# gnosisguild/stylus-zkvm-verifiers

Measured on AMD Instinct MI355X. Metric: Groth16 proofs verified/sec (BN254), higher is better.
Workload: dtype u32

## Files before the change

### stylus_zkvm_verifiers_amd/csrc/zkv_field.h

```cpp
#pragma once
#include <stdint.h>
#include "bn254_constants.h"

#if defined(__HIPCC__)
#define ZKV_HD __host__ __device__ __forceinline__
#define ZKV_HD_NI __host__ __device__ __noinline__ inline
#else
#define ZKV_HD inline
#define ZKV_HD_NI inline
#endif

#if defined(ZKV_COUNT_FP_MUL)
static thread_local unsigned long long zkv_fp_mul_counter = 0;
static thread_local unsigned long long zkv_mad_counter = 0;
#define ZKV_COUNT_MADS(n) (zkv_mad_counter += (n))
#else
#define ZKV_COUNT_MADS(n) ((void)0)
#endif

#if defined(__HIP_DEVICE_COMPILE__)
#define ZKV_TABLE static __device__ const
#else
#define ZKV_TABLE static const
#endif

#if defined(ZKV_ASM_MARKS) && defined(__HIP_DEVICE_COMPILE__)
#define ZKV_MARK(name) asm volatile("; ZKVMARK " name)
#else
#define ZKV_MARK(name) ((void)0)
#endif

#ifndef ZKV_FAIR_SLICE_SHIFT
#define ZKV_FAIR_SLICE_SHIFT 17
#endif
ZKV_HD uint32_t zkv_wave_slot_parity() {
#if defined(__HIP_DEVICE_COMPILE__) && !defined(ZKV_NO_FAIR_SHARE)
    return __builtin_amdgcn_s_getreg((3 << 11) | 4) & 1u;
#else
    return 0;
#endif
}
ZKV_HD void zkv_fair_share(uint32_t slot_parity) {
#if defined(__HIP_DEVICE_COMPILE__) && !defined(ZKV_NO_FAIR_SHARE)
    const uint32_t t = (uint32_t)(__builtin_amdgcn_s_memrealtime() >> ZKV_FAIR_SLICE_SHIFT);
    if ((t ^ slot_parity) & 1u) __builtin_amdgcn_s_setprio(1);
    else __builtin_amdgcn_s_setprio(0);
#else
    (void)slot_parity;
#endif
}

#include "zkv_modinv.h"

namespace zkv {

struct Fp { uint32_t v[8]; };
struct Fp2C { Fp c0, c1; };
#if defined(ZKV_PAIRED)
struct Fp2 { Fp h; };
#else
struct Fp2 { Fp c0, c1; };
#endif
struct Fp6 { Fp2 c0, c1, c2; };

#if defined(__has_builtin)
#if __has_builtin(__builtin_addc) && __has_builtin(__builtin_subc)
#define ZKV_HAVE_CARRY_BUILTINS 1
#endif
#endif
ZKV_HD uint32_t addc(uint32_t a, uint32_t b, uint32_t& carry) {
#if defined(ZKV_HAVE_CARRY_BUILTINS)
    unsigned co; uint32_t r = __builtin_addc(a, b, carry, &co); carry = co; return r;
#else
    uint64_t t = (uint64_t)a + b + carry;
    carry = (uint32_t)(t >> 32);
    return (uint32_t)t;
#endif
}
ZKV_HD uint32_t subb(uint32_t a, uint32_t b, uint32_t& borrow) {
#if defined(ZKV_HAVE_CARRY_BUILTINS)
    unsigned bo; uint32_t r = __builtin_subc(a, b, borrow, &bo); borrow = bo; return r;
#else
    uint64_t t = (uint64_t)a - b - borrow;
    borrow = (uint32_t)(t >> 32) & 1u;
    return (uint32_t)t;
#endif
}

ZKV_HD Fp fp_zero() { Fp r; for (int i = 0; i < 8; i++) r.v[i] = 0; return r; }
ZKV_HD Fp fp_one() { Fp r = ZKV_FP_ONE; return r; }
ZKV_HD bool fp_is_zero(const Fp& a) {
    const uint32_t P[8] = ZKV_FP_P_LIMBS;
    uint32_t o = 0, q = 0;
    for (int i = 0; i < 8; i++) { o |= a.v[i]; q |= a.v[i] ^ P[i]; }
    return o == 0 || q == 0;
}
ZKV_HD bool u256_geq(const uint32_t* a, const uint32_t* m) {
    uint32_t br = 0;
    for (int i = 0; i < 8; i++) (void)subb(a[i], m[i], br);
    return br == 0;
}
ZKV_HD Fp fp_add(const Fp& a, const Fp& b) {
    const uint32_t P[8] = ZKV_FP_2P_LIMBS;
    Fp t, s; uint32_t c = 0, br = 0;
#pragma unroll
    for (int i = 0; i < 8; i++) t.v[i] = addc(a.v[i], b.v[i], c);
#pragma unroll
    for (int i = 0; i < 8; i++) s.v[i] = subb(t.v[i], P[i], br);
#pragma unroll
    for (int i = 0; i < 8; i++) t.v[i] = br ? t.v[i] : s.v[i];
    return t;
}
ZKV_HD Fp fp_sub(const Fp& a, const Fp& b) {
    const uint32_t P[8] = ZKV_FP_2P_LIMBS;
    Fp t; uint32_t br = 0, c = 0;
#pragma unroll
    for (int i = 0; i < 8; i++) t.v[i] = subb(a.v[i], b.v[i], br);
    uint32_t mask = 0u - br;
#pragma unroll
    for (int i = 0; i < 8; i++) t.v[i] = addc(t.v[i], P[i] & mask, c);
    return t;
}
ZKV_HD bool fp_eq(const Fp& a, const Fp& b) { return fp_is_zero(fp_sub(a, b)); }
ZKV_HD Fp fp_neg(const Fp& a) { return fp_sub(fp_zero(), a); }
ZKV_HD Fp fp_dbl(const Fp& a) { return fp_add(a, a); }
ZKV_HD Fp fp_half(const Fp& a) {
    const uint32_t P[8] = ZKV_FP_P_LIMBS;
    const uint32_t m = 0u - (a.v[0] & 1u);
    Fp t; uint32_t c = 0;
#pragma unroll
    for (int i = 0; i < 8; i++) t.v[i] = addc(a.v[i], P[i] & m, c);
    Fp r;
#pragma unroll
    for (int i = 0; i < 7; i++) r.v[i] = (t.v[i] >> 1) | (t.v[i + 1] << 31);
    r.v[7] = t.v[7] >> 1;
    return r;
}
ZKV_HD Fp fp_add_nr(const Fp& a, const Fp& b) {
    Fp t; uint32_t c = 0;
#pragma unroll
    for (int i = 0; i < 8; i++) t.v[i] = addc(a.v[i], b.v[i], c);
    return t;
}
ZKV_HD void fp_add_x2(const Fp& a0, const Fp& b0, const Fp& a1, const Fp& b1, Fp& r0, Fp& r1) {
    const uint32_t P[8] = ZKV_FP_2P_LIMBS;
    Fp t0, t1, s0, s1; uint32_t c0 = 0, c1 = 0, w0 = 0, w1 = 0;
#pragma unroll
    for (int i = 0; i < 8; i++) { t0.v[i] = addc(a0.v[i], b0.v[i], c0); t1.v[i] = addc(a1.v[i], b1.v[i], c1); }
#pragma unroll
    for (int i = 0; i < 8; i++) { s0.v[i] = subb(t0.v[i], P[i], w0); s1.v[i] = subb(t1.v[i], P[i], w1); }
#pragma unroll
    for (int i = 0; i < 8; i++) { r0.v[i] = w0 ? t0.v[i] : s0.v[i]; r1.v[i] = w1 ? t1.v[i] : s1.v[i]; }
}
ZKV_HD void fp_sub_x2(const Fp& a0, const Fp& b0, const Fp& a1, const Fp& b1, Fp& r0, Fp& r1) {
    const uint32_t P[8] = ZKV_FP_2P_LIMBS;
    Fp t0, t1; uint32_t w0 = 0, w1 = 0, c0 = 0, c1 = 0;
#pragma unroll
    for (int i = 0; i < 8; i++) { t0.v[i] = subb(a0.v[i], b0.v[i], w0); t1.v[i] = subb(a1.v[i], b1.v[i], w1); }
    uint32_t m0 = 0u - w0, m1 = 0u - w1;
#pragma unroll
    for (int i = 0; i < 8; i++) { r0.v[i] = addc(t0.v[i], P[i] & m0, c0); r1.v[i] = addc(t1.v[i], P[i] & m1, c1); }
}

ZKV_HD void fp_unpack29(const Fp& a, uint32_t x[9]) {
#pragma unroll
    for (int k = 0; k < 9; k++) {
        const int bit = 29 * k, w = bit >> 5, s = bit & 31;
        uint32_t v = a.v[w] >> s;
        if (s > 3 && w < 7) v |= a.v[w + 1] << (32 - s);
        x[k] = v & 0x1fffffffu;
    }
}
template <typename COL>
ZKV_HD void fp_mac81(COL col[18], const uint32_t x[9], const uint32_t y[9]) {
    ZKV_COUNT_MADS(81);
#pragma unroll
    for (int i = 0; i < 9; i++) {
#pragma unroll
        for (int j = 0; j < 9; j++) col[i + j] = (COL)((uint64_t)col[i + j] + (uint64_t)x[i] * y[j]);
    }
}
template <typename COL>
ZKV_HD void fp_reduce_cols_limbs(COL col[18], uint32_t (&r)[9]) {
    ZKV_COUNT_MADS(81);
    const uint32_t P29[9] = ZKV_FP_P29_LIMBS;
    const uint32_t M29 = 0x1fffffffu;
#pragma unroll
    for (int i = 0; i < 9; i++) {
        uint32_t m = ((uint32_t)col[i] * ZKV_FP_INV29) & M29;
#pragma unroll
        for (int j = 0; j < 9; j++) col[i + j] = (COL)((uint64_t)col[i + j] + (uint64_t)m * P29[j]);
        col[i + 1] += col[i] >> 29;
    }
#pragma unroll
    for (int k = 9; k < 17; k++) {
        r[k - 9] = (uint32_t)col[k] & M29;
        col[k + 1] += col[k] >> 29;
    }
    r[8] = (uint32_t)col[17];
}
ZKV_HD Fp fp_pack29(const uint32_t (&r)[9]) {
    Fp o;
#pragma unroll
    for (int w = 0; w < 8; w++) {
        const int bit = 32 * w, k = bit / 29, s = bit - 29 * k, got = 29 - s;
        uint32_t v = r[k] >> s;
        if (k + 1 < 9) v |= r[k + 1] << got;
        if (got + 29 < 32 && k + 2 < 9) v |= r[k + 2] << (got + 29);
        o.v[w] = v;
    }
    return o;
}
template <typename COL>
ZKV_HD Fp fp_reduce_cols(COL col[18]) {
    uint32_t r[9];
    fp_reduce_cols_limbs(col, r);
    return fp_pack29(r);
}
#if defined(ZKV_FP_MUL_NOINLINE)
ZKV_HD_NI
#else
ZKV_HD
#endif
Fp fp_mul(Fp a, Fp b) {
#if defined(ZKV_COUNT_FP_MUL)
    zkv_fp_mul_counter++;
#endif
    uint32_t x[9], y[9];
    fp_unpack29(a, x); fp_unpack29(b, y);
    int64_t col[18];
#pragma unroll
    for (int k = 0; k < 18; k++) col[k] = 0;
    fp_mac81(col, x, y);
    return fp_reduce_cols(col);
}
#if defined(ZKV_FP_MUL_NOINLINE)
ZKV_HD_NI
#else
ZKV_HD
#endif
Fp fp_sqr(Fp a) {
#if defined(ZKV_COUNT_FP_MUL)
    zkv_fp_mul_counter++;
#endif
    uint32_t x[9], d[9];
    fp_unpack29(a, x);
#pragma unroll
    for (int i = 0; i < 9; i++) d[i] = x[i] << 1;
    uint64_t col[18];
    ZKV_COUNT_MADS(45);
#pragma unroll
    for (int k = 0; k < 18; k++) col[k] = 0;
#pragma unroll
    for (int i = 0; i < 9; i++) {
        col[2 * i] += (uint64_t)x[i] * x[i];
#pragma unroll
        for (int j = i + 1; j < 9; j++) col[i + j] += (uint64_t)d[i] * x[j];
    }
    return fp_reduce_cols(col);
}

ZKV_HD Fp fp_from_raw(const uint32_t* limbs) {
    Fp t, r2 = ZKV_FP_R2;
    for (int i = 0; i < 8; i++) t.v[i] = limbs[i];
    return fp_mul(t, r2);
}
ZKV_HD void fp_to_raw(uint32_t* limbs, const Fp& a) {
    const uint32_t P[8] = ZKV_FP_P_LIMBS;
    Fp one = fp_zero(); one.v[0] = 1;
    Fp t = fp_mul(a, one), s; uint32_t br = 0;
    for (int i = 0; i < 8; i++) s.v[i] = subb(t.v[i], P[i], br);
    for (int i = 0; i < 8; i++) limbs[i] = br ? t.v[i] : s.v[i];
}
ZKV_HD Fp fp_inv_fermat(const Fp& a) {
    const uint8_t S[ZKV_FP_INV_SCHED_LEN] = ZKV_FP_INV_SCHED;
    const Fp a3 = fp_mul(fp_sqr(a), a);
    Fp acc = (S[0] & 7) == 3 ? a3 : a;
#pragma unroll 1
    for (int i = 1; i < ZKV_FP_INV_SCHED_LEN; i++) {
        const int nsq = S[i] >> 3, v = S[i] & 7;
#pragma unroll 1
        for (int k = 0; k < nsq; k++) acc = fp_sqr(acc);
        if (v) {
            Fp m;
#pragma unroll
            for (int k = 0; k < 8; k++) m.v[k] = v == 3 ? a3.v[k] : a.v[k];
            acc = fp_mul(acc, m);
        }
    }
    return acc;
}

ZKV_HD Fp fp_inv(const Fp& a) {
    const int32_t M[9] = ZKV_FP_M30_LIMBS;
    const Fp r3 = ZKV_FP_R3;
    Fp t = a;
    modinv30(t.v, M, ZKV_FP_MINV30);
    return fp_mul(t, r3);
}

template <int N>
ZKV_HD void fp_add_n(const Fp (&a)[N], const Fp (&b)[N], Fp (&r)[N]) {
    const uint32_t P[8] = ZKV_FP_2P_LIMBS;
    Fp t[N], s[N]; uint32_t c[N], w[N];
#pragma unroll
    for (int k = 0; k < N; k++) { c[k] = 0; w[k] = 0; }
#pragma unroll
    for (int i = 0; i < 8; i++) {
#pragma unroll
        for (int k = 0; k < N; k++) t[k].v[i] = addc(a[k].v[i], b[k].v[i], c[k]);
    }
#pragma unroll
    for (int i = 0; i < 8; i++) {
#pragma unroll
        for (int k = 0; k < N; k++) s[k].v[i] = subb(t[k].v[i], P[i], w[k]);
    }
#pragma unroll
    for (int i = 0; i < 8; i++) {
#pragma unroll
        for (int k = 0; k < N; k++) r[k].v[i] = w[k] ? t[k].v[i] : s[k].v[i];
    }
}
template <int N>
ZKV_HD void fp_sub_n(const Fp (&a)[N], const Fp (&b)[N], Fp (&r)[N]) {
    const uint32_t P[8] = ZKV_FP_2P_LIMBS;
    Fp t[N]; uint32_t w[N], c[N], m[N];
#pragma unroll
    for (int k = 0; k < N; k++) { c[k] = 0; w[k] = 0; }
#pragma unroll
    for (int i = 0; i < 8; i++) {
#pragma unroll
        for (int k = 0; k < N; k++) t[k].v[i] = subb(a[k].v[i], b[k].v[i], w[k]);
    }
#pragma unroll
    for (int k = 0; k < N; k++) m[k] = 0u - w[k];
#pragma unroll
    for (int i = 0; i < 8; i++) {
#pragma unroll
        for (int k = 0; k < N; k++) r[k].v[i] = addc(t[k].v[i], P[i] & m[k], c[k]);
    }
// ... 81 lines not shown
    Fp r;
#pragma unroll
    for (int i = 0; i < 8; i++) r.v[i] = zkv_partner_u32(a.v[i]);
    return r;
}
ZKV_HD Fp fp_sel(bool odd, const Fp& if_odd, const Fp& if_even) {
    Fp r;
#pragma unroll
    for (int i = 0; i < 8; i++) r.v[i] = odd ? if_odd.v[i] : if_even.v[i];
    return r;
}
ZKV_HD Fp2 f2_const(const Fp2C& c) { Fp2 r; r.h = fp_sel(zkv_parity() != 0, c.c1, c.c0); return r; }
ZKV_HD Fp2 f2_zero() { Fp2 r; r.h = fp_zero(); return r; }
ZKV_HD Fp2 f2_one() { Fp2 r; r.h = fp_sel(zkv_parity() != 0, fp_zero(), fp_one()); return r; }
ZKV_HD bool f2_is_zero(const Fp2& a) {
    uint32_t o = fp_is_zero(a.h) ? 0u : 1u;
    o |= zkv_partner_u32(o);
    return o == 0;
}
ZKV_HD bool f2_eq(const Fp2& a, const Fp2& b) {
    uint32_t o = fp_eq(a.h, b.h) ? 0u : 1u;
    o |= zkv_partner_u32(o);
    return o == 0;
}
ZKV_HD Fp2 f2_add(const Fp2& a, const Fp2& b) { Fp2 r; r.h = fp_add(a.h, b.h); return r; }
ZKV_HD Fp2 f2_sub(const Fp2& a, const Fp2& b) { Fp2 r; r.h = fp_sub(a.h, b.h); return r; }
ZKV_HD Fp2 f2_neg(const Fp2& a) { Fp2 r; r.h = fp_neg(a.h); return r; }
ZKV_HD Fp2 f2_add_nr(const Fp2& a, const Fp2& b) { Fp2 r; r.h = fp_add_nr(a.h, b.h); return r; }
ZKV_HD Fp2 f2_dbl(const Fp2& a) { return f2_add(a, a); }
ZKV_HD Fp2 f2_half(const Fp2& a) { Fp2 r; r.h = fp_half(a.h); return r; }
ZKV_HD Fp2 f2_conj(const Fp2& a) { Fp2 r; r.h = fp_sel(zkv_parity() != 0, fp_neg(a.h), a.h); return r; }
#if defined(ZKV_FP_MUL_NOINLINE)
ZKV_HD_NI
#else
ZKV_HD
#endif
Fp f2_mul_lane(Fp my_a, Fp my_b) {
#if defined(ZKV_COUNT_FP_MUL)
    zkv_fp_mul_counter += 2;
#endif
    const uint32_t FAT[9] = ZKV_FP_FAT8P_LIMBS;
    const bool odd = zkv_parity() != 0;
    uint32_t xa[9], xo[9], yb[9], U[9], V[9];
    fp_unpack29(my_a, xa); fp_unpack29(my_b, yb);
#pragma unroll
    for (int i = 0; i < 9; i++) { xo[i] = zkv_partner_u32(xa[i]); U[i] = zkv_pair_even_u32(yb[i]); V[i] = zkv_pair_odd_u32(yb[i]); }
    if (!odd) {
#pragma unroll
        for (int i = 0; i < 9; i++) V[i] = FAT[i] - V[i];
    }
    uint64_t col[18];
#pragma unroll
    for (int k = 0; k < 18; k++) col[k] = 0;
    fp_mac81(col, xa, U); fp_mac81(col, xo, V);
    return fp_reduce_cols(col);
}
ZKV_HD Fp2 f2_mul(const Fp2& a, const Fp2& b) { Fp2 r; r.h = f2_mul_lane(a.h, b.h); return r; }
ZKV_HD void f2_limbs_x(const Fp& v, uint32_t (&own)[9], uint32_t (&par)[9]) {
    fp_unpack29(v, own);
#pragma unroll
    for (int i = 0; i < 9; i++) par[i] = zkv_partner_u32(own[i]);
}
ZKV_HD void f2_limbs_y(const Fp& v, uint32_t (&U)[9], uint32_t (&V)[9]) {
    const uint32_t FAT[9] = ZKV_FP_FAT8P_LIMBS;
    uint32_t y[9];
    fp_unpack29(v, y);
#pragma unroll
    for (int i = 0; i < 9; i++) { U[i] = zkv_pair_even_u32(y[i]); V[i] = zkv_pair_odd_u32(y[i]); }
    if (zkv_parity() == 0) {
#pragma unroll
        for (int i = 0; i < 9; i++) V[i] = FAT[i] - V[i];
    }
}
ZKV_HD Fp f2_dot2_limbs(const uint32_t (&ao)[9], const uint32_t (&ap)[9], const uint32_t (&bU)[9], const uint32_t (&bV)[9],
                        const uint32_t (&co)[9], const uint32_t (&cp)[9], const uint32_t (&dU)[9], const uint32_t (&dV)[9]) {
#if defined(ZKV_COUNT_FP_MUL)
    zkv_fp_mul_counter += 4;
#endif
    uint64_t col[18];
#pragma unroll
    for (int k = 0; k < 18; k++) col[k] = 0;
    fp_mac81(col, ao, bU); fp_mac81(col, ap, bV); fp_mac81(col, co, dU); fp_mac81(col, cp, dV);
    return fp_reduce_cols(col);
}
ZKV_HD Fp f2_mul_limbs(const uint32_t (&ao)[9], const uint32_t (&ap)[9], const uint32_t (&bU)[9], const uint32_t (&bV)[9]) {
#if defined(ZKV_COUNT_FP_MUL)
    zkv_fp_mul_counter += 2;
#endif
    uint64_t col[18];
#pragma unroll
    for (int k = 0; k < 18; k++) col[k] = 0;
    fp_mac81(col, ao, bU); fp_mac81(col, ap, bV);
    return fp_reduce_cols(col);
}
struct L9 { uint32_t l[9]; };
ZKV_HD L9 l9_from_fp(const Fp& a) { L9 r; fp_unpack29(a, r.l); return r; }
ZKV_HD Fp l9_to_fp(const L9& a) { return fp_pack29(a.l); }
ZKV_HD L9 l9_partner(const L9& a) {
    L9 r;
#pragma unroll
    for (int i = 0; i < 9; i++) r.l[i] = zkv_partner_u32(a.l[i]);
    return r;
}
ZKV_HD L9 l9_mul_core(const L9& a, const L9& b) {
#if defined(ZKV_COUNT_FP_MUL)
    zkv_fp_mul_counter += 2;
#endif
    const uint32_t FAT[9] = ZKV_FP_FAT8P_LIMBS;
    uint32_t xo[9], U[9], V[9];
    uint64_t col[18];
#pragma unroll
    for (int k = 0; k < 18; k++) col[k] = 0;
#pragma unroll
    for (int i = 0; i < 9; i++) U[i] = zkv_pair_even_u32(b.l[i]);
    fp_mac81(col, a.l, U);
#pragma unroll
    for (int i = 0; i < 9; i++) { xo[i] = zkv_partner_u32(a.l[i]); V[i] = zkv_pair_odd_u32(b.l[i]); }
    if (zkv_parity() == 0) {
#pragma unroll
        for (int i = 0; i < 9; i++) V[i] = FAT[i] - V[i];
    }
    fp_mac81(col, xo, V);
    L9 r; fp_reduce_cols_limbs(col, r.l);
    return r;
}
#if defined(__HIP_DEVICE_COMPILE__) && defined(ZKV_FP_MUL_NOINLINE)
#define ZKV_L9P(p) uint32_t p##0, uint32_t p##1, uint32_t p##2, uint32_t p##3, uint32_t p##4, uint32_t p##5, uint32_t p##6, uint32_t p##7, uint32_t p##8
#define ZKV_L9A(f) f.l[0], f.l[1], f.l[2], f.l[3], f.l[4], f.l[5], f.l[6], f.l[7], f.l[8]
#define ZKV_L9MK(f, p) L9 f; f.l[0] = p##0; f.l[1] = p##1; f.l[2] = p##2; f.l[3] = p##3; f.l[4] = p##4; f.l[5] = p##5; f.l[6] = p##6; f.l[7] = p##7; f.l[8] = p##8
__device__ __noinline__ inline L9 l9_mul_ni(ZKV_L9P(pa), ZKV_L9P(pb)) {
    ZKV_L9MK(a, pa); ZKV_L9MK(b, pb);
    return l9_mul_core(a, b);
}
ZKV_HD L9 l9_mul(const L9& a, const L9& b) { return l9_mul_ni(ZKV_L9A(a), ZKV_L9A(b)); }
#else
ZKV_HD L9 l9_mul(const L9& a, const L9& b) { return l9_mul_core(a, b); }
#endif
struct LTerm { const uint32_t* x; int32_t k; };
#define ZKV_L9_G 256
template <int N> ZKV_HD L9 l9_lincomb(const LTerm (&t)[N], const int c) {
    const uint32_t P29[9] = ZKV_FP_P29_LIMBS;
    const int32_t D = (int32_t)P29[8] + 1;
    const uint32_t M = (uint32_t)(((1ull << 53) + (uint64_t)D - 1) / (uint64_t)D);
    int32_t top = 0;
#pragma unroll
    for (int j = 0; j < N; j++) top += t[j].k * (int32_t)t[j].x[8];
    const uint32_t tt = (uint32_t)(top + c * D - c - ZKV_L9_G);
    const int32_t nq = c - (int32_t)(uint32_t)(((uint64_t)tt * M) >> 53);
    L9 y; int64_t carry = 0;
#pragma unroll
    for (int i = 0; i < 9; i++) {
        int64_t s = carry;
#pragma unroll
        for (int j = 0; j < N; j++) s += (int64_t)t[j].k * (int64_t)(int32_t)t[j].x[i];
        s += (int64_t)nq * (int64_t)(int32_t)P29[i];
        if (i < 8) { y.l[i] = (uint32_t)s & 0x1fffffffu; carry = s >> 29; }
        else y.l[i] = (uint32_t)s;
    }
    return y;
}
ZKV_HD Fp2 f2_sqr(const Fp2& a) {
    const bool odd = zkv_parity() != 0;
    Fp o = zkv_partner(a.h);
    Fp x = fp_add_nr(a.h, fp_sel(odd, a.h, o));
    Fp y = fp_sel(odd, o, fp_sub(a.h, o));
    Fp2 r; r.h = fp_mul(x, y);
// ... 94 lines not shown
```

### stylus_zkvm_verifiers_amd/csrc/zkv_tower_mem.h

```cpp
#pragma once
#include "zkv_curve.h"

namespace zkv {

struct MRef {
    uint32_t* p; uint32_t stride; uint32_t f2w;
    ZKV_HD uint32_t ld(int k) const { return p[(size_t)k * stride]; }
    ZKV_HD void st(int k, uint32_t v) const { p[(size_t)k * stride] = v; }
    ZKV_HD int fw() const { return (int)f2w; }
};
ZKV_HD MRef m_ref(uint32_t* p, uint32_t stride, uint32_t f2w = 16) { MRef r; r.p = p; r.stride = stride; r.f2w = f2w; return r; }
ZKV_HD MRef m_off(MRef m, int words) { MRef r = m; r.p = m.p + (size_t)words * m.stride; return r; }

struct SoaRW {
    uint32_t* p; size_t stride; uint32_t off;
    ZKV_HD uint32_t ld(int k) const { return *(const uint32_t*)((const char*)(p + (size_t)k * stride) + off); }
    ZKV_HD void st(int k, uint32_t v) const { *(uint32_t*)((char*)(p + (size_t)k * stride) + off) = v; }
    ZKV_HD int fw() const { return 16; }
};
template <class R> ZKV_HD R m_fresh(R r) { return r; }
ZKV_HD SoaRW m_fresh(SoaRW r) {
#if defined(__HIP_DEVICE_COMPILE__)
    asm volatile("" : "+v"(r.off));
#endif
    return r;
}

#if defined(__HIP_DEVICE_COMPILE__)
typedef __attribute__((address_space(3))) uint32_t zkv_lds_u32;
#else
typedef uint32_t zkv_lds_u32;
#endif
struct LRef {
    zkv_lds_u32* p;
    ZKV_HD uint32_t ld(int k) const { return p[k * 64]; }
    ZKV_HD void st(int k, uint32_t v) const { p[k * 64] = v; }
#if defined(ZKV_PAIRED)
    ZKV_HD int fw() const { return 8; }
#else
    ZKV_HD int fw() const { return 16; }
#endif
};
ZKV_HD LRef l_ref(uint32_t* lds_base_plus_lane) { LRef r; r.p = (zkv_lds_u32*)lds_base_plus_lane; return r; }

template <class R> ZKV_HD Fp m_ld_fp(R m, int word0) {
    Fp r;
#pragma unroll
    for (int k = 0; k < 8; k++) r.v[k] = m.ld(word0 + k);
    return r;
}
template <class R> ZKV_HD void m_st_fp(R m, int word0, const Fp& a) {
#pragma unroll
    for (int k = 0; k < 8; k++) m.st(word0 + k, a.v[k]);
}
#if defined(ZKV_PAIRED)
template <class R> ZKV_HD Fp2 m_ld_f2(R m, int idx) { Fp2 r; r.h = m_ld_fp(m, m.fw() * idx); return r; }
template <class R> ZKV_HD void m_st_f2(R m, int idx, const Fp2& a) { m_st_fp(m, m.fw() * idx, a.h); }
#else
template <class R> ZKV_HD Fp2 m_ld_f2(R m, int idx) { Fp2 r; r.c0 = m_ld_fp(m, 16 * idx); r.c1 = m_ld_fp(m, 16 * idx + 8); return r; }
template <class R> ZKV_HD void m_st_f2(R m, int idx, const Fp2& a) { m_st_fp(m, 16 * idx, a.c0); m_st_fp(m, 16 * idx + 8, a.c1); }
#endif
template <class R> ZKV_HD Fp6 m_ld_f6(R m, int idx) { Fp6 r; r.c0 = m_ld_f2(m, idx); r.c1 = m_ld_f2(m, idx + 1); r.c2 = m_ld_f2(m, idx + 2); return r; }
template <class R> ZKV_HD void m_st_f6(R m, int idx, const Fp6& a) { m_st_f2(m, idx, a.c0); m_st_f2(m, idx + 1, a.c1); m_st_f2(m, idx + 2, a.c2); }
template <class RD, class RA> ZKV_HD void f12m_copy(RD d, RA a) {
#pragma unroll 1
    for (int k = 0; k < 6; k++) m_st_f2(d, k, m_ld_f2(a, k));
}
template <class RD> ZKV_HD void f12m_set_one(RD d) {
    m_st_f2(d, 0, f2_one());
#pragma unroll 1
    for (int k = 1; k < 6; k++) m_st_f2(d, k, f2_zero());
}
template <class RD> ZKV_HD void f12m_conj(RD d) {
#pragma unroll 1
    for (int k = 3; k < 6; k++) m_st_f2(d, k, f2_neg(m_ld_f2(d, k)));
}
template <class RA> ZKV_HD bool f12m_is_one(RA a) {
    bool ok = f2_eq(m_ld_f2(a, 0), f2_one());
#pragma unroll 1
    for (int k = 1; k < 6; k++) ok = f2_is_zero(m_ld_f2(a, k)) && ok;
    return ok;
}

template <class RF> ZKV_HD void f12m_sqr_body(RF f) {
    Fp6 g = m_ld_f6(f, 0), h = m_ld_f6(f, 3);
    Fp6 t = f6_mul(g, h);
    Fp6 s = f6_mul(f6_add(g, h), f6_add(g, f6_mul_v(h)));
    m_st_f6(f, 0, f6_sub(f6_sub(s, t), f6_mul_v(t)));
    m_st_f6(f, 3, f6_add(t, t));
}
template <class RF> ZKV_HD_NI void f12m_sqr(RF f) { f12m_sqr_body(f); }
ZKV_HD void fp4_sqr(const Fp2& a, const Fp2& b, Fp2& t0, Fp2& t1) {
    Fp2 tmp = f2_mul(a, b);
    t0 = f2_sub(f2_sub(f2_mul(f2_add(a, b), f2_add(f2_mul_xi(b), a)), tmp), f2_mul_xi(tmp));
    t1 = f2_dbl(tmp);
}
template <class RF> ZKV_HD void f12m_cyclo_sqr_body(RF f) {
    Fp2 z0 = m_ld_f2(f, 0), z1 = m_ld_f2(f, 4), t0, t1;
    fp4_sqr(z0, z1, t0, t1);
    z0 = f2_sub(t0, z0); z0 = f2_add(f2_dbl(z0), t0);
    z1 = f2_add(t1, z1); z1 = f2_add(f2_dbl(z1), t1);
    m_st_f2(f, 0, z0); m_st_f2(f, 4, z1);
    Fp2 z2 = m_ld_f2(f, 3), z3 = m_ld_f2(f, 2), t2, t3;
    fp4_sqr(z2, z3, t2, t3);
    Fp2 z4 = m_ld_f2(f, 1), z5 = m_ld_f2(f, 5), t4, t5;
    fp4_sqr(z4, z5, t4, t5);
    Fp2 x = f2_mul_xi(t5);
    z2 = f2_add(x, z2); z2 = f2_add(f2_dbl(z2), x);
    z3 = f2_sub(t4, z3); z3 = f2_add(f2_dbl(z3), t4);
    z4 = f2_sub(t2, z4); z4 = f2_add(f2_dbl(z4), t2);
    z5 = f2_add(t3, z5); z5 = f2_add(f2_dbl(z5), t3);
    m_st_f2(f, 3, z2); m_st_f2(f, 2, z3); m_st_f2(f, 1, z4); m_st_f2(f, 5, z5);
}
template <class RF> ZKV_HD_NI void f12m_cyclo_sqr(RF f) { f12m_cyclo_sqr_body(f); }
#if defined(ZKV_PAIRED)
struct L9Ref {
    zkv_lds_u32* p;
    ZKV_HD int fw() const { return 8; }
};
ZKV_HD L9Ref l9_ref(uint32_t* lds_base_plus_lane) { L9Ref r; r.p = (zkv_lds_u32*)lds_base_plus_lane; return r; }
ZKV_HD L9 l9_ld(L9Ref m, int idx) {
    L9 r;
#pragma unroll
    for (int k = 0; k < 9; k++) r.l[k] = m.p[(9 * idx + k) * 64];
    return r;
}
ZKV_HD void l9_st(L9Ref m, int idx, const L9& a) {
#pragma unroll
    for (int k = 0; k < 9; k++) m.p[(9 * idx + k) * 64] = a.l[k];
}
ZKV_HD Fp m_ld_fp(L9Ref m, int word0) { return l9_to_fp(l9_ld(m, word0 >> 3)); }
ZKV_HD void m_st_fp(L9Ref m, int word0, const Fp& a) { l9_st(m, word0 >> 3, l9_from_fp(a)); }

ZKV_HD void l9_fp4_sqr_update(const L9& a, const L9& b, const L9& za, const L9& zb, const bool xi_t1, L9& o0, L9& o1) {
    const bool odd = zkv_parity() != 0;
    const int32_t k1 = odd ? 1 : -1, k3 = odd ? -3 : 3;
    const L9 tmp = l9_mul(a, b);
    L9 s1, s2;
#pragma unroll
    for (int i = 0; i < 9; i++) s1.l[i] = a.l[i] + b.l[i];
    {
        const L9 pb = l9_partner(b);
        const LTerm t[3] = {{a.l, 1}, {b.l, 9}, {pb.l, k1}};
// ... 118 lines not shown
        const RB S = m_fresh(S0);
        l9_f6_mul_raw([&](int i) { return l9_ld(acc, 3 + i); }, [&](int i) {
            Fp2 b = m_ld_f2(S, 3 + i);
            if (conj_b) b = f2_neg(b);
            return l9_from_fp(f2_add(m_ld_f2(S, i), b).h);
        }, raw);
        l9_partner_i32(raw.wa, pw);
        { const LTerm t[4] = {{raw.v0.l, 1}, {(const uint32_t*)raw.wa, 9}, {(const uint32_t*)pw, k1}, {xy0, -1}}; h0 = l9_lincomb(t, 52); }
        const L9 pv2 = l9_partner(raw.v2);
        { const LTerm t[4] = {{(const uint32_t*)raw.wb, 1}, {raw.v2.l, 9}, {pv2.l, k1}, {xy1, -1}}; h1 = l9_lincomb(t, 12); }
        { const LTerm t[2] = {{(const uint32_t*)raw.wc, 1}, {xy2, -1}}; h2 = l9_lincomb(t, 12); }
    }
    l9_st(acc, 3, h0); l9_st(acc, 4, h1); l9_st(acc, 5, h2);
}
ZKV_HD void l9_pin(L9& a) {
#if defined(__HIP_DEVICE_COMPILE__)
#pragma unroll
    for (int i = 0; i < 9; i++) asm volatile("" : "+v"(a.l[i]));
#else
    (void)a;
#endif
}
template <class RB> ZKV_HD void f12l9_mul_aw(L9Ref acc, RB S0, const bool neg, const bool keep) {
    const int32_t k1 = zkv_parity() != 0 ? 1 : -1;
    const int32_t sg = neg ? -1 : 1, sg9 = 9 * sg, sgk = k1 * sg;
    L9F6Raw raw;
    int32_t pw[9];
    L9 n0, n1, n2;
    {
        const RB S = m_fresh(S0);
        l9_f6_mul_raw([&](int i) { return l9_ld(acc, i); }, [&](int i) { return l9_from_fp(m_ld_f2(S, i).h); }, raw);
        l9_partner_i32(raw.wa, pw);
        const L9 d2 = l9_ld(acc, 5), pd2 = l9_partner(d2);
        { const LTerm t[5] = {{raw.v0.l, sg}, {(const uint32_t*)raw.wa, sg9}, {(const uint32_t*)pw, sgk}, {d2.l, 9}, {pd2.l, k1}}; n0 = l9_lincomb(t, 48); }
        const L9 pv2 = l9_partner(raw.v2), d0 = l9_ld(acc, 3);
        { const LTerm t[4] = {{(const uint32_t*)raw.wb, sg}, {raw.v2.l, sg9}, {pv2.l, sgk}, {d0.l, 1}}; n1 = l9_lincomb(t, 28); }
        const L9 d1 = l9_ld(acc, 4);
        { const LTerm t[2] = {{(const uint32_t*)raw.wc, sg}, {d1.l, 1}}; n2 = l9_lincomb(t, 8); }
    }
    l9_pin(n0); l9_pin(n1); l9_pin(n2);
    L9 h0, h1, h2;
    {
        const RB S = m_fresh(S0);
        l9_f6_mul_raw([&](int i) { return l9_ld(acc, 3 + i); }, [&](int i) { return l9_from_fp(m_ld_f2(S, i).h); }, raw);
        l9_partner_i32(raw.wa, pw);
        const L9 g0 = l9_ld(acc, 0);
        { const LTerm t[4] = {{raw.v0.l, sg}, {(const uint32_t*)raw.wa, sg9}, {(const uint32_t*)pw, sgk}, {g0.l, 1}}; h0 = l9_lincomb(t, 48); }
        const L9 pv2 = l9_partner(raw.v2), g1 = l9_ld(acc, 1);
        { const LTerm t[4] = {{(const uint32_t*)raw.wb, sg}, {raw.v2.l, sg9}, {pv2.l, sgk}, {g1.l, 1}}; h1 = l9_lincomb(t, 28); }
        const L9 g2 = l9_ld(acc, 2);
        { const LTerm t[2] = {{(const uint32_t*)raw.wc, sg}, {g2.l, 1}}; h2 = l9_lincomb(t, 8); }
    }
    if (keep) {
        l9_st(acc, 0, n0); l9_st(acc, 1, n1); l9_st(acc, 2, n2);
        l9_st(acc, 3, h0); l9_st(acc, 4, h1); l9_st(acc, 5, h2);
    }
}
template <class RA, class RT> ZKV_HD bool f12m_eq_conj(RA a, RT t) {
    bool ok = true;
#pragma unroll 1
    for (int k = 0; k < 6; k++) {
        const Fp2 x = m_ld_f2(a, k), y = m_ld_f2(t, k);
        ok = (k < 3 ? f2_eq(x, y) : f2_is_zero(f2_add(x, y))) && ok;
    }
    return ok;
}
#endif

template <class RD, class RA, class RB> ZKV_HD void f12m_mul_body(RD d, RA a, RB b, bool conj_b) {
    Fp6 ag = m_ld_f6(a, 0), bg = m_ld_f6(b, 0);
    Fp6 t0 = f6_mul(ag, bg);
    Fp6 ah = m_ld_f6(a, 3), bh = m_ld_f6(b, 3);
    if (conj_b) bh = f6_neg(bh);
    Fp6 t1 = f6_mul(ah, bh);
    Fp6 m = f6_mul(f6_add(ag, ah), f6_add(bg, bh));
    d = m_fresh(d);
    m_st_f6(d, 3, f6_sub(f6_sub(m, t0), t1));
    m_st_f6(d, 0, f6_add(t0, f6_mul_v(t1)));
}
template <class RD, class RA, class RB> ZKV_HD_NI void f12m_mul(RD d, RA a, RB b) { f12m_mul_body(d, a, b, false); }
template <class RD, class RA, class RB> ZKV_HD_NI void f12m_mul_conj(RD d, RA a, RB b) { f12m_mul_body(d, a, b, true); }
#if defined(ZKV_PAIRED)
template <class RF> ZKV_HD void f12m_mul_by_034_body(RF f, const Fp2& c0, const Fp2& c3, const Fp2& c4) {
    uint32_t c0U[9], c0V[9], c4U[9], c4V[9], tU[9], tV[9], xo[9], xp[9];
    f2_limbs_y(c0.h, c0U, c0V); f2_limbs_y(c4.h, c4U, c4V);
    Fp2 t0c0, t0c1, t0c2, t1c0, t1c1, t1c2;
    {
        const Fp2 h0 = m_ld_f2(f, 3), h1 = m_ld_f2(f, 4), h2 = m_ld_f2(f, 5);
        Fp2 p4, p5, p6, p7, p8;
        f2_limbs_y(c3.h, tU, tV);
        f2_limbs_x(h0.h, xo, xp); p4.h = f2_mul_limbs(xo, xp, tU, tV);
        f2_limbs_x(h2.h, xo, xp); p8.h = f2_mul_limbs(xo, xp, tU, tV); p7.h = f2_mul_limbs(xo, xp, c4U, c4V);
        f2_limbs_x(h1.h, xo, xp); p5.h = f2_mul_limbs(xo, xp, c4U, c4V);
        f2_limbs_y(f2_add_nr(c3, c4).h, tU, tV);
        f2_limbs_x(f2_add_nr(h0, h1).h, xo, xp); p6.h = f2_mul_limbs(xo, xp, tU, tV);
        t1c0 = f2_add(p4, f2_mul_xi(p7)); t1c1 = f2_sub(f2_sub(p6, p4), p5); t1c2 = f2_add(p5, p8);
    }
    Fp2 s0, s1, s2;
    {
        const Fp2 g0 = m_ld_f2(f, 0), g1 = m_ld_f2(f, 1), g2 = m_ld_f2(f, 2);
        f2_limbs_x(g0.h, xo, xp); t0c0.h = f2_mul_limbs(xo, xp, c0U, c0V);
        f2_limbs_x(g1.h, xo, xp); t0c1.h = f2_mul_limbs(xo, xp, c0U, c0V);
        f2_limbs_x(g2.h, xo, xp); t0c2.h = f2_mul_limbs(xo, xp, c0U, c0V);
        s0 = f2_add(g0, m_ld_f2(f, 3)); s1 = f2_add(g1, m_ld_f2(f, 4)); s2 = f2_add(g2, m_ld_f2(f, 5));
    }
    m_st_f2(f, 0, f2_add(t0c0, f2_mul_xi(t1c2))); m_st_f2(f, 1, f2_add(t0c1, t1c0)); m_st_f2(f, 2, f2_add(t0c2, t1c1));
    const Fp2 b0 = f2_add(c0, c3);
    Fp2 w0, w1, n, q;
    f2_limbs_y(b0.h, tU, tV);
    f2_limbs_x(s0.h, xo, xp); w0.h = f2_mul_limbs(xo, xp, tU, tV);
    f2_limbs_x(s2.h, xo, xp); q.h = f2_mul_limbs(xo, xp, tU, tV);
    Fp2 q2; q2.h = f2_mul_limbs(xo, xp, c4U, c4V);
    f2_limbs_x(s1.h, xo, xp); w1.h = f2_mul_limbs(xo, xp, c4U, c4V);
    f2_limbs_y(f2_add_nr(b0, c4).h, tU, tV);
    f2_limbs_x(f2_add_nr(s0, s1).h, xo, xp); n.h = f2_mul_limbs(xo, xp, tU, tV);
    m_st_f2(f, 3, f2_sub(f2_sub(f2_add(w0, f2_mul_xi(q2)), t0c0), t1c0));
    m_st_f2(f, 4, f2_sub(f2_sub(f2_sub(f2_sub(n, w0), w1), t0c1), t1c1));
    m_st_f2(f, 5, f2_sub(f2_sub(f2_add(w1, q), t0c2), t1c2));
}
#else
template <class RF> ZKV_HD void f12m_mul_by_034_body(RF f, const Fp2& c0, const Fp2& c3, const Fp2& c4) {
    Fp6 g = m_ld_f6(f, 0), h = m_ld_f6(f, 3);
    Fp6 t0 = f6_mul_fp2(g, c0);
    Fp6 t1 = f6_mul_by_01(h, c3, c4);
    Fp6 t2 = f6_mul_by_01(f6_add(g, h), f2_add(c0, c3), c4);
    m_st_f6(f, 3, f6_sub(f6_sub(t2, t0), t1));
    m_st_f6(f, 0, f6_add(t0, f6_mul_v(t1)));
}
#endif
template <class RF> ZKV_HD_NI void f12m_mul_by_034(RF f, const Fp2* c0, const Fp2* c3, const Fp2* c4) { f12m_mul_by_034_body(f, *c0, *c3, *c4); }
#if defined(ZKV_PAIRED)
template <class RF> ZKV_HD void f12m_mul_by_134_body(RF f, const Fp2& c3, const Fp2& c4) {
    uint32_t c3U[9], c3V[9], c4U[9], c4V[9], x3U[9], x3V[9], x4U[9], x4V[9];
    f2_limbs_y(c3.h, c3U, c3V); f2_limbs_y(c4.h, c4U, c4V);
    { const Fp2 x3 = f2_mul_xi(c3), x4 = f2_mul_xi(c4); f2_limbs_y(x3.h, x3U, x3V); f2_limbs_y(x4.h, x4U, x4V); }
    Fp ng0, ng1, ng2, nh0, nh1, nh2;
    {
        uint32_t h0o[9], h0p[9], h1o[9], h1p[9], h2o[9], h2p[9];
        f2_limbs_x(m_ld_f2(f, 3).h, h0o, h0p); f2_limbs_x(m_ld_f2(f, 4).h, h1o, h1p); f2_limbs_x(m_ld_f2(f, 5).h, h2o, h2p);
        ng0 = fp_add(m_ld_f2(f, 0).h, f2_dot2_limbs(h1o, h1p, x4U, x4V, h2o, h2p, x3U, x3V));
        ng1 = fp_add(m_ld_f2(f, 1).h, f2_dot2_limbs(h0o, h0p, c3U, c3V, h2o, h2p, x4U, x4V));
        ng2 = fp_add(m_ld_f2(f, 2).h, f2_dot2_limbs(h0o, h0p, c4U, c4V, h1o, h1p, c3U, c3V));
    }
    {
        uint32_t g0o[9], g0p[9], g1o[9], g1p[9], g2o[9], g2p[9];
        f2_limbs_x(m_ld_f2(f, 0).h, g0o, g0p); f2_limbs_x(m_ld_f2(f, 1).h, g1o, g1p); f2_limbs_x(m_ld_f2(f, 2).h, g2o, g2p);
        nh0 = fp_add(m_ld_f2(f, 3).h, f2_dot2_limbs(g0o, g0p, c3U, c3V, g2o, g2p, x4U, x4V));
        nh1 = fp_add(m_ld_f2(f, 4).h, f2_dot2_limbs(g0o, g0p, c4U, c4V, g1o, g1p, c3U, c3V));
        nh2 = fp_add(m_ld_f2(f, 5).h, f2_dot2_limbs(g1o, g1p, c4U, c4V, g2o, g2p, c3U, c3V));
    }
    Fp2 o;
    o.h = ng0; m_st_f2(f, 0, o); o.h = ng1; m_st_f2(f, 1, o); o.h = ng2; m_st_f2(f, 2, o);
    o.h = nh0; m_st_f2(f, 3, o); o.h = nh1; m_st_f2(f, 4, o); o.h = nh2; m_st_f2(f, 5, o);
}
#else
template <class RF> ZKV_HD void f12m_mul_by_134_body(RF f, const Fp2& c3, const Fp2& c4) {
    Fp6 g = m_ld_f6(f, 0), h = m_ld_f6(f, 3);
    Fp6 hs = f6_mul_by_01(h, c3, c4);
    Fp6 gs = f6_mul_by_01(g, c3, c4);
    m_st_f6(f, 0, f6_add(g, f6_mul_v(hs)));
    m_st_f6(f, 3, f6_add(h, gs));
}
#endif
template <class RF> ZKV_HD_NI void f12m_mul_by_134(RF f, const Fp2* c3, const Fp2* c4) { f12m_mul_by_134_body(f, *c3, *c4); }
template <class RD, class RA> ZKV_HD void f12m_inv_body(RD d, RA a) {
    Fp6 g = m_ld_f6(a, 0), h = m_ld_f6(a, 3);
// ... 40 lines not shown
```

Baseline: 6.723 million.

## Compute sparse Fp12 mul_by_034 as fused three-term Fp2 dot products

Replaces the Karatsuba-style sparse multiply-by-034 in the Miller loop with a schoolbook formulation. Each output Fp2 coefficient is built from three accumulated products sharing a single Montgomery reduction, using an intermediate 32-bit column carry so six products fit in 64-bit columns. This removes the Karatsuba pre-additions and several separate reductions, at the cost of more raw multiply-accumulates and higher register pressure. It also adds scheduling pins and careful load/store ordering so the update can happen in place, plus host-only overflow shadow checks.

```diff
diff --git a/stylus_zkvm_verifiers_amd/csrc/zkv_field.h b/stylus_zkvm_verifiers_amd/csrc/zkv_field.h
--- a/stylus_zkvm_verifiers_amd/csrc/zkv_field.h
+++ b/stylus_zkvm_verifiers_amd/csrc/zkv_field.h
@@ -13,9 +13,12 @@
 #if defined(ZKV_COUNT_FP_MUL)
 static thread_local unsigned long long zkv_fp_mul_counter = 0;
 static thread_local unsigned long long zkv_mad_counter = 0;
-#define ZKV_COUNT_MADS(n) (zkv_mad_counter += (n))
+static thread_local unsigned long long zkv_mad_issued_counter = 0;
+#define ZKV_COUNT_MADS(n) (zkv_mad_counter += (n), zkv_mad_issued_counter += (n))
+#define ZKV_COUNT_MADS_ISSUED(n) (zkv_mad_issued_counter += (n))
 #else
 #define ZKV_COUNT_MADS(n) ((void)0)
+#define ZKV_COUNT_MADS_ISSUED(n) ((void)0)
 #endif
 
 #if defined(__HIP_DEVICE_COMPILE__)
@@ -171,13 +174,31 @@
         x[k] = v & 0x1fffffffu;
     }
 }
+#if defined(ZKV_SHADOW_COLS) && !defined(__HIP_DEVICE_COMPILE__)
+static thread_local unsigned long long zkv_col_shadow_ops = 0, zkv_col_shadow_bad = 0;
+inline void zkv_col_shadow(uint64_t c, uint64_t t) {
+    zkv_col_shadow_ops++;
+    if ((unsigned __int128)c + (unsigned __int128)t != (unsigned __int128)(uint64_t)(c + t)) zkv_col_shadow_bad++;
+}
+inline void zkv_col_shadow(int64_t c, __int128 t) {
+    zkv_col_shadow_ops++;
+    if ((__int128)c + t != (__int128)(int64_t)((uint64_t)c + (uint64_t)(int64_t)t)) zkv_col_shadow_bad++;
+}
+#define ZKV_COL_SHADOW(c, t) zkv_col_shadow(c, t)
+#else
+#define ZKV_COL_SHADOW(c, t) ((void)0)
+#endif
+ZKV_HD uint64_t col_add(uint64_t c, uint64_t t) { ZKV_COL_SHADOW(c, t); return c + t; }
+ZKV_HD int64_t col_add(int64_t c, uint64_t t) { ZKV_COL_SHADOW(c, (__int128)t); return (int64_t)((uint64_t)c + t); }
+ZKV_HD uint64_t col_carry(uint64_t c, uint64_t carry) { ZKV_COL_SHADOW(c, carry); return c + carry; }
+ZKV_HD int64_t col_carry(int64_t c, int64_t carry) { ZKV_COL_SHADOW(c, (__int128)carry); return (int64_t)((uint64_t)c + (uint64_t)carry); }
 template <typename COL>
 ZKV_HD void fp_mac81(COL col[18], const uint32_t x[9], const uint32_t y[9]) {
     ZKV_COUNT_MADS(81);
 #pragma unroll
     for (int i = 0; i < 9; i++) {
 #pragma unroll
-        for (int j = 0; j < 9; j++) col[i + j] = (COL)((uint64_t)col[i + j] + (uint64_t)x[i] * y[j]);
+        for (int j = 0; j < 9; j++) col[i + j] = col_add(col[i + j], (uint64_t)x[i] * y[j]);
     }
 }
 template <typename COL>
@@ -189,13 +210,13 @@
     for (int i = 0; i < 9; i++) {
         uint32_t m = ((uint32_t)col[i] * ZKV_FP_INV29) & M29;
 #pragma unroll
-        for (int j = 0; j < 9; j++) col[i + j] = (COL)((uint64_t)col[i + j] + (uint64_t)m * P29[j]);
-        col[i + 1] += col[i] >> 29;
+        for (int j = 0; j < 9; j++) col[i + j] = col_add(col[i + j], (uint64_t)m * P29[j]);
+        col[i + 1] = col_carry(col[i + 1], (COL)(col[i] >> 29));
     }
 #pragma unroll
     for (int k = 9; k < 17; k++) {
         r[k - 9] = (uint32_t)col[k] & M29;
-        col[k + 1] += col[k] >> 29;
+        col[k + 1] = col_carry(col[k + 1], (COL)(col[k] >> 29));
     }
     r[8] = (uint32_t)col[17];
 }
@@ -253,9 +274,9 @@
     for (int k = 0; k < 18; k++) col[k] = 0;
 #pragma unroll
     for (int i = 0; i < 9; i++) {
-        col[2 * i] += (uint64_t)x[i] * x[i];
-#pragma unroll
-        for (int j = i + 1; j < 9; j++) col[i + j] += (uint64_t)d[i] * x[j];
+        col[2 * i] = col_add(col[2 * i], (uint64_t)x[i] * x[i]);
+#pragma unroll
+        for (int j = i + 1; j < 9; j++) col[i + j] = col_add(col[i + j], (uint64_t)d[i] * x[j]);
     }
     return fp_reduce_cols(col);
 }
@@ -503,6 +524,57 @@
     for (int k = 0; k < 18; k++) col[k] = 0;
     fp_mac81(col, ao, bU); fp_mac81(col, ap, bV); fp_mac81(col, co, dU); fp_mac81(col, cp, dV);
     return fp_reduce_cols(col);
+}
+ZKV_HD void fp_cols_carry32(uint64_t (&col)[18]) {
+    uint32_t eight = 8u;
+#if defined(__HIP_DEVICE_COMPILE__)
+    asm volatile("" : "+s"(eight));
+#endif
+#pragma unroll
+    for (int k = 17; k >= 1; k--) {
+        const uint32_t hi = (uint32_t)(col[k - 1] >> 32);
+        uint64_t keep = k == 17 ? col[17] : (uint64_t)(uint32_t)col[k];
+        ZKV_COUNT_MADS_ISSUED(1);
+        col[k] = col_add(keep, (uint64_t)hi * eight);
+#if defined(__HIP_DEVICE_COMPILE__)
+        asm volatile("" : "+v"(col[k]));
+#endif
+    }
+    col[0] = (uint64_t)(uint32_t)col[0];
+}
+#if defined(ZKV_SHADOW_COLS) && !defined(__HIP_DEVICE_COMPILE__)
+inline void zkv_dot3_operands(const uint32_t (&xo)[9], const uint32_t (&xp)[9], const uint32_t (&U)[9], const uint32_t (&V)[9]) {
+    for (int i = 0; i < 9; i++)
+        if ((xo[i] >> 29) || (xp[i] >> 29) || (U[i] >> 29) || (V[i] >> 30)) zkv_col_shadow_bad++;
+}
+#define ZKV_DOT3_OPERANDS(a, b, c, d) zkv_dot3_operands(a, b, c, d)
+#else
+#define ZKV_DOT3_OPERANDS(a, b, c, d) ((void)0)
+#endif
+ZKV_HD void f2_dot3_first(uint64_t (&col)[18], const uint32_t (&ao)[9], const uint32_t (&ap)[9], const uint32_t (&bU)[9], const uint32_t (&bV)[9],
+                          const uint32_t (&co)[9], const uint32_t (&cp)[9], const uint32_t (&dU)[9], const uint32_t (&dV)[9]) {
+#if defined(ZKV_COUNT_FP_MUL)
+    zkv_fp_mul_counter += 4;
+#endif
+    ZKV_DOT3_OPERANDS(ao, ap, bU, bV); ZKV_DOT3_OPERANDS(co, cp, dU, dV);
+#pragma unroll
+    for (int k = 0; k < 18; k++) col[k] = 0;
+    fp_mac81(col, ao, bU); fp_mac81(col, ap, bV); fp_mac81(col, co, dU); fp_mac81(col, cp, dV);
+    fp_cols_carry32(col);
+}
+ZKV_HD Fp f2_dot3_last(uint64_t (&col)[18], const uint32_t (&eo)[9], const uint32_t (&ep)[9], const uint32_t (&fU)[9], const uint32_t (&fV)[9]) {
+#if defined(ZKV_COUNT_FP_MUL)
+    zkv_fp_mul_counter += 2;
+#endif
+    ZKV_DOT3_OPERANDS(eo, ep, fU, fV);
+    fp_mac81(col, eo, fU); fp_mac81(col, ep, fV);
+    Fp r = fp_reduce_cols(col);
+#if defined(__HIP_DEVICE_COMPILE__)
+#pragma unroll
+    for (int k = 0; k < 8; k++) asm volatile("" : "+v"(r.v[k]));
+    __builtin_amdgcn_sched_barrier(0);
+#endif
+    return r;
 }
 ZKV_HD Fp f2_mul_limbs(const uint32_t (&ao)[9], const uint32_t (&ap)[9], const uint32_t (&bU)[9], const uint32_t (&bV)[9]) {
 #if defined(ZKV_COUNT_FP_MUL)
diff --git a/stylus_zkvm_verifiers_amd/csrc/zkv_tower_mem.h b/stylus_zkvm_verifiers_amd/csrc/zkv_tower_mem.h
--- a/stylus_zkvm_verifiers_amd/csrc/zkv_tower_mem.h
+++ b/stylus_zkvm_verifiers_amd/csrc/zkv_tower_mem.h
@@ -59,6 +59,28 @@
 #else
 template <class R> ZKV_HD Fp2 m_ld_f2(R m, int idx) { Fp2 r; r.c0 = m_ld_fp(m, 16 * idx); r.c1 = m_ld_fp(m, 16 * idx + 8); return r; }
 template <class R> ZKV_HD void m_st_f2(R m, int idx, const Fp2& a) { m_st_fp(m, 16 * idx, a.c0); m_st_fp(m, 16 * idx + 8, a.c1); }
+#endif
+#if defined(ZKV_PAIRED)
+template <class R> ZKV_HD R m_again(R r) { return r; }
+ZKV_HD LRef m_again(LRef r) {
+#if defined(__HIP_DEVICE_COMPILE__)
+    asm volatile("" : "+v"(r.p));
+#endif
+    return r;
+}
+ZKV_HD void f2_pin(Fp2& a) {
+#if defined(__HIP_DEVICE_COMPILE__)
+#pragma unroll
+    for (int k = 0; k < 8; k++) asm volatile("" : "+v"(a.h.v[k]));
+#else
+    (void)a;
+#endif
+}
+template <class R> ZKV_HD Fp2 m_ld_f2_again(R m, int idx) {
+    Fp2 r = m_ld_f2(m_again(m), idx);
+    f2_pin(r);
+    return r;
+}
 #endif
 template <class R> ZKV_HD Fp6 m_ld_f6(R m, int idx) { Fp6 r; r.c0 = m_ld_f2(m, idx); r.c1 = m_ld_f2(m, idx + 1); r.c2 = m_ld_f2(m, idx + 2); return r; }
 template <class R> ZKV_HD void m_st_f6(R m, int idx, const Fp6& a) { m_st_f2(m, idx, a.c0); m_st_f2(m, idx + 1, a.c1); m_st_f2(m, idx + 2, a.c2); }
@@ -343,6 +365,47 @@
 template <class RD, class RA, class RB> ZKV_HD_NI void f12m_mul_conj(RD d, RA a, RB b) { f12m_mul_body(d, a, b, true); }
 #if defined(ZKV_PAIRED)
 template <class RF> ZKV_HD void f12m_mul_by_034_body(RF f, const Fp2& c0, const Fp2& c3, const Fp2& c4) {
+    uint32_t lU[9], lV[9], aU[9], aV[9], bU[9], bV[9];
+    f2_limbs_y(c0.h, lU, lV); f2_limbs_y(c3.h, aU, aV); f2_limbs_y(c4.h, bU, bV);
+    uint32_t g0o[9], g0p[9], g1o[9], g1p[9], g2o[9], g2p[9], h0o[9], h0p[9], h1o[9], h1p[9], h2o[9], h2p[9];
+    uint64_t col[18];
+    Fp2 nh1, nh2, o;
+    f2_limbs_x(m_ld_f2(f, 2).h, g2o, g2p); f2_limbs_x(m_ld_f2(f, 1).h, g1o, g1p);
+    f2_dot3_first(col, g2o, g2p, aU, aV, g1o, g1p, bU, bV);
+    f2_limbs_x(m_ld_f2(f, 5).h, h2o, h2p);
+    nh2.h = f2_dot3_last(col, h2o, h2p, lU, lV);
+    f2_limbs_x(m_ld_f2(f, 0).h, g0o, g0p);
+    f2_dot3_first(col, g1o, g1p, aU, aV, g0o, g0p, bU, bV);
+    f2_limbs_x(m_ld_f2(f, 4).h, h1o, h1p);
+    nh1.h = f2_dot3_last(col, h1o, h1p, lU, lV);
+    f2_dot3_first(col, h1o, h1p, aU, aV, g2o, g2p, lU, lV);
+    f2_limbs_x(m_ld_f2(f, 3).h, h0o, h0p);
+    o.h = f2_dot3_last(col, h0o, h0p, bU, bV);
+    {
+        Fp2 nh0, x4 = f2_mul_xi(c4);
+        f2_dot3_first(col, g0o, g0p, aU, aV, h0o, h0p, lU, lV);
+        f2_pin(x4); f2_limbs_y(x4.h, bU, bV);
+        nh0.h = f2_dot3_last(col, g2o, g2p, bU, bV);
+        m_st_f2(f, 2, o);
+        f2_limbs_x(m_ld_f2_again(f, 5).h, h2o, h2p);
+        m_st_f2(f, 5, nh2);
+        f2_dot3_first(col, h0o, h0p, aU, aV, h2o, h2p, bU, bV);
+        f2_limbs_x(m_ld_f2_again(f, 1).h, g1o, g1p);
+        o.h = f2_dot3_last(col, g1o, g1p, lU, lV);
+        m_st_f2(f, 3, nh0); m_st_f2(f, 1, o);
+    }
+    { const Fp2 x3 = f2_mul_xi(c3); f2_limbs_y(x3.h, aU, aV); }
+    f2_limbs_x(m_ld_f2_again(f, 4).h, h1o, h1p);
+    m_st_f2(f, 4, nh1);
+    f2_dot3_first(col, h2o, h2p, aU, aV, h1o, h1p, bU, bV);
+    f2_limbs_x(m_ld_f2_again(f, 0).h, g0o, g0p);
+    o.h = f2_dot3_last(col, g0o, g0p, lU, lV);
+    m_st_f2(f, 0, o);
+#if defined(ZKV_COUNT_FP_MUL)
+    zkv_fp_mul_counter -= 10; zkv_mad_counter -= 243;
+#endif
+}
+template <class RF> ZKV_HD void f12m_mul_by_034_karatsuba_body(RF f, const Fp2& c0, const Fp2& c3, const Fp2& c4) {
     uint32_t c0U[9], c0V[9], c4U[9], c4V[9], tU[9], tV[9], xo[9], xp[9];
     f2_limbs_y(c0.h, c0U, c0V); f2_limbs_y(c4.h, c4U, c4V);
     Fp2 t0c0, t0c1, t0c2, t1c0, t1c1, t1c2;
```

After: 6.869 million, median of 6. 1.02x the previous value.
